# gyroflow/gyroflow

Hardware: NVIDIA H100
Metric: 4K frames/sec (fisheye+RS warp) (higher is better)
Workload: dtype f32

## Files before the change

gyroflow_b200/abi.py:

```python
import ctypes as C
import os

_HERE = os.path.dirname(os.path.abspath(__file__))
LIB_PATH = os.environ.get("GF_CUDA_LIB") or os.path.join(_HERE, "libgyroflow_cuda.so")

MATRIX_STRIDE = 14
MESH_MAX_LEN = 839
KERNEL_PARAMS_SIZE = 368


class KernelParams(C.Structure):
    _pack_ = 4
    _fields_ = [
        ("width", C.c_int32), ("height", C.c_int32), ("stride", C.c_int32),
        ("output_width", C.c_int32), ("output_height", C.c_int32), ("output_stride", C.c_int32),
        ("matrix_count", C.c_int32), ("interpolation", C.c_int32), ("background_mode", C.c_int32),
        ("flags", C.c_int32), ("bytes_per_pixel", C.c_int32), ("pix_element_count", C.c_int32),
        ("background", C.c_float * 4), ("f", C.c_float * 2), ("c", C.c_float * 2), ("k", C.c_float * 12),
        ("fov", C.c_float), ("r_limit", C.c_float), ("lens_correction_amount", C.c_float),
        ("input_vertical_stretch", C.c_float), ("input_horizontal_stretch", C.c_float),
        ("background_margin", C.c_float), ("background_margin_feather", C.c_float), ("canvas_scale", C.c_float),
        ("input_rotation", C.c_float), ("output_rotation", C.c_float),
        ("translation2d", C.c_float * 2), ("translation3d", C.c_float * 4),
        ("source_rect", C.c_int32 * 4), ("output_rect", C.c_int32 * 4),
# ... 136 lines not shown
    ("gf_lens_from_name", C.c_int, [C.c_char_p]),
    ("gf_lens_name", C.c_char_p, [C.c_int]),
    ("gf_pixel_bytes", C.c_int, [C.c_int]),
    ("gf_combo_supported", C.c_int, [C.c_int, C.c_int, C.c_int, C.c_int]),
    ("gf_cuda_create", C.c_int, [_P(C.c_void_p), C.c_int, _P(KernelParams), C.c_int, C.c_int, C.c_int,
                                 _P(BufferDesc), _P(BufferDesc), C.c_size_t]),
    ("gf_cuda_destroy", None, [C.c_void_p]),
    ("gf_cuda_undistort_image", C.c_int, [C.c_void_p, _P(BufferDesc), _P(BufferDesc), _P(KernelParams),
                                          C.c_void_p, C.c_size_t, C.c_void_p, C.c_size_t,
                                          C.c_void_p, C.c_size_t, C.c_void_p]),
    ("gf_cuda_undistort_image_dev", C.c_int, [C.c_void_p, _P(BufferDesc), _P(BufferDesc), _P(KernelParams),
                                              C.c_void_p, C.c_size_t, C.c_void_p, C.c_size_t, C.c_void_p]),
    ("gf_cuda_undistort_image_async", C.c_int, [C.c_void_p, _P(BufferDesc), _P(BufferDesc), _P(KernelParams),
                                                C.c_void_p, C.c_size_t, C.c_void_p, C.c_size_t, C.c_void_p]),
    ("gf_cuda_validate_tables_dev", C.c_int, [C.c_void_p, C.c_void_p, C.c_size_t]),
    ("gf_cuda_undistort_points", C.c_int, [C.c_void_p, C.c_void_p, C.c_int, C.c_int, C.c_double, C.c_size_t, C.c_int, C.c_double, C.c_void_p, C.c_size_t, C.c_void_p, C.c_void_p]),
    ("gf_cuda_stmap_distort_dev", C.c_int, [C.c_void_p, C.c_void_p, C.c_int, C.c_int, C.c_double, C.c_size_t, C.c_void_p, C.c_void_p]),
    ("gf_cuda_generate_stmap", C.c_int, [C.c_void_p, C.c_void_p, C.c_int, C.c_int, C.c_int, C.c_size_t, C.c_double, C.POINTER(C.c_int32), C.POINTER(C.c_int32),
                                          C.c_void_p, C.c_size_t, C.c_void_p, C.c_size_t, C.c_void_p]),
    ("gf_cuda_undistort_planes_dev", C.c_int, [C.c_void_p, C.c_size_t, C.c_void_p, C.c_void_p, C.c_void_p, C.c_void_p, C.c_size_t, C.c_void_p, C.c_size_t, C.c_void_p]),
    ("gf_cuda_undistort_planes", C.c_int, [C.c_void_p, C.c_size_t, C.c_void_p, C.c_void_p, C.c_void_p, C.c_void_p, C.c_size_t, C.c_void_p, C.c_size_t, C.c_void_p]),
    ("gf_cuda_selftest_exhaustive", C.c_int, [C.c_int, C.POINTER(C.c_ulonglong)]),
    ("gf_cuda_selftest_filter", C.c_int, [C.c_int, C.c_ulonglong, C.c_int, C.c_int, C.POINTER(C.c_ulonglong)]),
    ("gf_cuda_plan", C.c_int, [C.c_void_p, C.c_int, C.c_int, C.c_int, C.c_void_p, C.c_void_p, C.c_size_t, C.c_uint32, C.c_size_t]),
    ("gf_cuda_synchronize", C.c_int, [C.c_void_p]),
    ("gf_cuda_set_overlays", C.c_int, [C.c_void_p, C.c_int]),
    ("gf_cuda_last_error", C.c_char_p, [C.c_void_p]),
    ("gf_cuda_backend_name", C.c_char_p, []),
    ("gf_cuda_launch_count", C.c_uint64, [C.c_void_p]),
    ("gf_cuda_selftest", C.c_int, [C.c_int, C.c_ulonglong, C.c_ulonglong, _P(C.c_ulonglong)]),
    ("gf_frame_transform_at_timestamp", C.c_int, [_P(ComputeParams), C.c_double, C.c_size_t, _P(KernelParams), C.c_void_p, C.c_size_t,
                                                  _P(C.c_size_t), _P(C.c_double), _P(C.c_double)]),
    ("gf_cuda_gyro_upload", C.c_int, [_P(C.c_void_p), C.c_int, _P(ComputeParams)]),
    ("gf_cuda_gyro_free", None, [C.c_void_p]),
    ("gf_cuda_frame_transform_dev", C.c_int, [C.c_void_p, _P(ComputeParams), C.c_double, C.c_size_t, _P(KernelParams), C.c_void_p, C.c_size_t,
                                              _P(C.c_size_t), _P(C.c_double), _P(C.c_double), C.c_void_p]),
    ("gf_cuda_find_fovs", C.c_int, [C.c_void_p, _P(ComputeParams), C.c_int, C.c_int, C.c_void_p, C.c_size_t, C.c_float, C.c_void_p, C.c_void_p]),
    ("gf_zoom_dynamic_compute", C.c_int, [C.c_void_p, C.c_size_t, C.c_double, C.c_double, C.c_int, C.c_void_p]),
    ("gf_zoom_fovs", C.c_int, [_P(ZoomParams), C.c_void_p, C.c_void_p, C.c_size_t, C.c_void_p, C.c_void_p]),
    ("gf_cuda_calculate_fovs", C.c_int, [C.c_void_p, _P(ComputeParams), _P(ZoomParams), C.c_int, C.c_int, C.c_void_p, C.c_size_t,
                                         C.c_void_p, C.c_void_p, C.c_void_p]),
    ("gf_cuda_scan_tables_dev", C.c_int, [C.c_void_p, C.c_size_t, C.c_void_p, C.c_void_p]),
    ("gf_cuda_undistort_image_dev_flagged", C.c_int, [C.c_void_p, _P(BufferDesc), _P(BufferDesc), _P(KernelParams),
                                                      C.c_void_p, C.c_size_t, C.c_void_p, C.c_size_t, C.c_void_p, C.c_void_p]),
    ("gf_cuda_undistort_planes_dev_flagged", C.c_int, [C.c_void_p, C.c_size_t, C.c_void_p, C.c_void_p, C.c_void_p, C.c_void_p, C.c_size_t,
                                                       C.c_void_p, C.c_size_t, C.c_void_p, C.c_void_p]),
# ... 45 lines not shown
```

gyroflow_b200/csrc/c_abi.cu:

```cuda
#include <cuda_runtime.h>
#include <cstdio>
#include <cstring>
#include <cstdlib>
#include <mutex>
#include <cmath>
#include <algorithm>
#include <string>
#include <vector>

#include "kernel_registry.h"
#include "c_abi_internal.h"
#include <nvtx3/nvToolsExt.h>

using namespace gf;

namespace {

struct Slot {
    GrowBuf<float, true> h_mat, h_mesh;
    GrowBuf<float> d_mat, d_mesh;
    GrowBuf<double> d_mesh64;
    Event done;
};
constexpr int kSlots = 4;
// ... 165 lines not shown
    }
    A.feat = f;

    for (int i = 0; i < 4; ++i) A.bg[i] = p->background[i] * p->max_pixel_value;
    const float factor = fmaxf(1.0f - p->lens_correction_amount, 0.001f);
    A.out_c[0] = (float)p->output_width / 2.0f; A.out_c[1] = (float)p->output_height / 2.0f;
    A.out_f[0] = p->f[0] / p->fov / factor;      A.out_f[1] = p->f[1] / p->fov / factor;

    A.width_f = (float)p->width; A.height_f = (float)p->height;
    A.frame_w = A.width_f; A.frame_h = A.height_f;
    A.rot_cos = 1.0f; A.rot_sin = 0.0f;
    if (p->input_rotation != 0.0f) {
        const float rotation = p->input_rotation * (3.14159274101257324f / 180.0f);
        A.rot_cos = gf_cosf(rotation); A.rot_sin = gf_sinf(rotation);
        const float fx = A.rot_cos * (A.width_f - 0.0f) - A.rot_sin * (A.height_f - 0.0f) + 0.0f;
        const float fy = A.rot_sin * (A.width_f - 0.0f) + A.rot_cos * (A.height_f - 0.0f) + 0.0f;
        A.frame_w = rs_round(fabsf(fx)); A.frame_h = rs_round(fabsf(fy));
    }
    A.omap_x = make_map((float)p->output_rect[0], (float)(p->output_rect[0] + p->output_rect[2]), 0.0f, (float)p->output_width,  (float)A.out_cols);
    A.omap_y = make_map((float)p->output_rect[1], (float)(p->output_rect[1] + p->output_rect[3]), 0.0f, (float)p->output_height, (float)A.out_rows);
    A.smap_x = make_map(0.0f, A.frame_w, (float)p->source_rect[0], (float)(p->source_rect[0] + p->source_rect[2]), -1.0f);
    A.smap_y = make_map(0.0f, A.frame_h, (float)p->source_rect[1], (float)(p->source_rect[1] + p->source_rect[3]), -1.0f);
    A.rs_lim = (p->flags & 16) == 16 ? p->width : p->height;
    const float lim = p->pixel_value_limit;
    A.u8_limit = (lim != lim) ? 255 : (lim < 0.0f ? 0 : (lim >= 255.0f ? 255 : (int)lim));
    A.src_rect[0] = p->source_rect[0]; A.src_rect[1] = p->source_rect[1];
    A.src_rect[2] = p->source_rect[0] + p->source_rect[2]; A.src_rect[3] = p->source_rect[1] + p->source_rect[3];
    A.interior_span[0] = A.src_rect[2] - 2 - A.src_rect[0]; A.interior_span[1] = A.src_rect[3] - 2 - A.src_rect[1];
    if (A.interior_span[0] < 0 || A.interior_span[1] < 0 || A.interior_span[0] >= (1 << 17) || A.interior_span[1] >= (1 << 17) || A.rs_lim >= (1 << 22)) { A.interior_span[0] = 0; A.interior_span[1] = 0; A.feat |= F_WILD; }
    auto smap_ok = [](const MapC& m) { return m.fast_div && m.in_min == 0.0f && m.mul != 0.0f && tame(m.mul) && m.div > 0.0f && m.div <= 0x1p20f && std::isfinite(m.add) && fabsf(m.add) <= 0x1p16f; };
    if (!(smap_ok(A.smap_x) && smap_ok(A.smap_y) && fabsf(p->c[0]) >= 0x1p-10f && fabsf(p->c[1]) >= 0x1p-10f &&
          A.src_rect[0] >= 0 && A.src_rect[1] >= 0 && A.src_rect[2] <= (1 << 16) && A.src_rect[3] <= (1 << 16))) A.feat |= F_WILD;
    auto int_map_ok = [](const MapC& m) {
        return m.identity || (m.fast_div && m.mul > 0.0f && m.div > 0.0f && tame(m.mul) && std::isfinite(m.add) && fabsf(m.in_min) <= 0x1p20f);
    };
    if (!(int_map_ok(A.omap_x) && int_map_ok(A.omap_y))) A.feat |= F_WILD;
    A.hot.rect[0] = A.src_rect[0]; A.hot.rect[1] = A.src_rect[1]; A.hot.rect[2] = A.interior_span[0]; A.hot.rect[3] = A.interior_span[1];
    if (A.omap_x.identity && A.omap_y.identity && A.omap_x.add == truncf(A.omap_x.add) && A.omap_y.add == truncf(A.omap_y.add) &&
        fabsf(A.omap_x.add) < 0x1p20f && fabsf(A.omap_y.add) < 0x1p20f && fabsf(A.omap_x.in_min) < 0x1p20f && fabsf(A.omap_y.in_min) < 0x1p20f) {
        A.hot.x_off = (int)A.omap_x.add - (int)A.omap_x.in_min; A.hot.y_off = (int)A.omap_y.add - (int)A.omap_y.in_min;
        A.hot.x0 = std::max(0, -A.hot.x_off); A.hot.x1 = std::min(A.out_cols, p->output_width - A.hot.x_off);
        A.hot.y0 = std::max(0, -A.hot.y_off); A.hot.y1 = std::min(A.out_rows, p->output_height - A.hot.y_off);
        A.hot.full_rows = (int)std::min<size_t>(A.dst_len / (size_t)p->output_stride, (size_t)A.out_rows);
        const size_t tail = A.dst_len - (size_t)A.hot.full_rows * (size_t)p->output_stride;
        A.hot.last_cols = (A.hot.full_rows < A.out_rows) ? (int)std::min<size_t>(tail / (size_t)bpp, (size_t)A.out_cols) : 0;
        A.feat |= F_INTPRO;
    }
}

float filter_a_cap(const float* k) {
    auto B = [&](double t) { const double t2 = t * t; return t2 * (fabs((double)k[0]) + t2 * (fabs((double)k[1]) + t2 * (fabs((double)k[2]) + t2 * fabs((double)k[3])))); };
    for (int i = 0; i < 4; ++i) if (!std::isfinite(k[i])) return 0.0f;
    double lo = 0.0, hi = 1.55;
    if (B(hi) > 0.25) { for (int it = 0; it < 60; ++it) { const double mid = 0.5 * (lo + hi); if (B(mid) <= 0.25) lo = mid; else hi = mid; } }
    else lo = hi;
    if (lo < 0.5) return 0.0f;
    const double a = tan(lo) * tan(lo);
    return (float)std::min(a * 0.999, 16000.0);
}

struct FrameJob {
    const gf_buffer_desc* in; const gf_buffer_desc* out; const gf_kernel_params* p;
    const float* matrices; size_t matrix_rows;
    const float* mesh; size_t mesh_len;
    void* stream;
    bool tables_on_device = false;
    bool sync_host = true;
    size_t more_planes = 0;
// ... 604 lines not shown
```

gyroflow_b200/csrc/selftest.cu:

```cuda
#include <cuda_runtime.h>
#include <cstdio>
#include <cstdlib>
#include <cstring>
#include <cmath>
#include <vector>
#include "../../include/gyroflow_cuda.h"
#include "warp_kernel_x2.cuh"
#include "c_abi_internal.h"

using namespace gf;

namespace {
inline uint32_t __float_as_uint_host(float f) { uint32_t u; memcpy(&u, &f, 4); return u; }
__device__ __forceinline__ uint32_t mix(uint64_t v) {
    v ^= v >> 33; v *= 0xff51afd7ed558ccdULL; v ^= v >> 33; v *= 0xc4ceb9fe1a85ec53ULL; v ^= v >> 33;
    return (uint32_t)v;
}
__device__ __forceinline__ float gen(uint64_t i, uint32_t salt) {
    const uint32_t h = mix(i * 0x9E3779B97F4A7C15ULL + salt);
    const uint32_t sel = mix(i + 77u * salt) & 7u;
    if (sel < 3) return __uint_as_float(h);
    if (sel < 6) return __uint_as_float((h & 0x807fffffu) | ((100u + (mix(i ^ salt) % 56u)) << 23));
    return __uint_as_float((h & 0x007fffffu) | 0x3f800000u) - ((h >> 31) ? 0.0f : 1.0f);
}
// ... 92 lines not shown
    unsigned long long in_regime = 0, violations = 0, uncertain = 0; unsigned worst = 0;
    for (int ci = blockIdx.y; ci < n_cfg; ci += gridDim.y) {
        const FilterCfg C = cfgs[ci];
        gf_kernel_params P; memset(&P, 0, sizeof(P));
        for (int i = 0; i < 4; ++i) P.k[i] = C.k[i];
        P.f[0] = C.f1; P.f[1] = C.f1; P.c[0] = 0.5f * (float)C.w; P.c[1] = C.c1;
        const int nx = (C.w + step - 1) / step, ny = (C.h + step - 1) / step;
        for (int i = blockIdx.x * blockDim.x + threadIdx.x; i < nx * ny; i += gridDim.x * blockDim.x) {
            const float px = (float)((i % nx) * step + (ci % step)), py = (float)((i / nx) * step + ((ci / 3) % step));
            const float _x = (px * C.m[0] + py * C.m[1]) + C.m[2];
            const float _y = (px * C.m[3] + py * C.m[4]) + C.m[5];
            const float _w = (px * C.m[6] + py * C.m[7]) + C.m[8];
            float tvc;
            if (!Lens2<GF_LENS_OPENCV_FISHEYE>::approx_v(_x, _y, _w, P, C.a_cap, tvc)) continue;
            const float tv = tvc + P.c[1];
            if (!(fabsf(tv) < 0x1p20f)) continue;
            float ex, ey;
            Lens<GF_LENS_OPENCV_FISHEYE>::distort(_x, _y, _w, P, false, ex, ey);
            const float tv_exact = ey * P.f[1] + P.c[1];
            const float bound = __fmaf_rn(fabsf(tvc), rho, fabsf(tv) * 0x1p-22f);
            const float diff = fabsf(tv - tv_exact);
            ++in_regime;
            if (!(diff <= bound)) ++violations;
            const float z = tv - 0.5f;
            if (!(fabsf(z - ((z + 12582912.0f) - 12582912.0f)) > bound)) ++uncertain;
            const float ratio = bound > 0.0f ? diff / bound : (diff > 0.0f ? 1e9f : 0.0f);
            worst = max(worst, (unsigned)fminf(ratio * 1e6f, 4.0e9f));
        }
    }
    if (in_regime) atomicAdd(&out[0], in_regime);
    if (violations) atomicAdd(&out[1], violations);
    if (uncertain) atomicAdd(&out[2], uncertain);
    atomicMax(&out[3], (unsigned long long)worst);
}
}

extern "C" GF_API int gf_cuda_selftest_filter(int device, unsigned long long seed, int n_cfg, int step, unsigned long long* out4) {
    if (!out4 || n_cfg < 1 || step < 1) return GF_ERR_BAD_PARAMS;
    CK(nullptr, cudaSetDevice(device));
    std::vector<FilterCfg> cfgs((size_t)n_cfg);
    uint64_t st = seed * 0x9E3779B97F4A7C15ULL + 12345u;
    auto rnd = [&]() { st ^= st << 13; st ^= st >> 7; st ^= st << 17; return (double)(st >> 11) * (1.0 / 9007199254740992.0); };
    for (int i = 0; i < n_cfg; ++i) {
        FilterCfg& C = cfgs[(size_t)i];
        const int sizes[5][2] = { {3840, 2160}, {1920, 1080}, {7680, 4320}, {1280, 720}, {8192, 4320} };
        C.w = sizes[i % 5][0]; C.h = sizes[i % 5][1];
        double k[4]; for (int j = 0; j < 4; ++j) k[j] = (rnd() * 2.0 - 1.0) * pow(0.35, j);
        const double t_hit = 0.6 + 0.95 * rnd(), t2 = t_hit * t_hit;
// ... 6 lines not shown
        const double f = (0.3 + 0.9 * rnd()) * C.w, cx = 0.5 * C.w, cy = 0.5 * C.h;
        double ax[3] = { rnd() - 0.5, rnd() - 0.5, rnd() - 0.5 }; const double an = sqrt(ax[0]*ax[0] + ax[1]*ax[1] + ax[2]*ax[2]) + 1e-12;
        for (double& v : ax) v /= an;
        const double ang = 0.45 * rnd(), c = cos(ang), s = sin(ang), t = 1.0 - c;
        const double R[9] = { t*ax[0]*ax[0] + c, t*ax[0]*ax[1] - s*ax[2], t*ax[0]*ax[2] + s*ax[1],
                              t*ax[0]*ax[1] + s*ax[2], t*ax[1]*ax[1] + c, t*ax[1]*ax[2] - s*ax[0],
                              t*ax[0]*ax[2] - s*ax[1], t*ax[1]*ax[2] + s*ax[0], t*ax[2]*ax[2] + c };
        const double Ki[9] = { 1.0 / f, 0.0, -cx / f, 0.0, 1.0 / f, -cy / f, 0.0, 0.0, 1.0 };
        for (int r = 0; r < 3; ++r) for (int q = 0; q < 3; ++q) C.m[r * 3 + q] = (float)(R[0 * 3 + r] * Ki[0 * 3 + q] + R[1 * 3 + r] * Ki[1 * 3 + q] + R[2 * 3 + r] * Ki[2 * 3 + q]);
        C.f1 = (float)((0.3 + 0.9 * rnd()) * C.w); C.c1 = (float)(cy + (rnd() - 0.5) * 40.0);
    }
    GrowBuf<FilterCfg> d_cfg; GrowBuf<unsigned long long> d_out;
    CK(nullptr, d_cfg.reserve(cfgs.size(), nullptr));
    CK(nullptr, d_out.reserve(4, nullptr));
    CK(nullptr, cudaMemcpy(d_cfg.ptr, cfgs.data(), cfgs.size() * sizeof(FilterCfg), cudaMemcpyHostToDevice));
    CK(nullptr, cudaMemset(d_out.ptr, 0, 4 * sizeof(unsigned long long)));
    filter_check_kernel<<<dim3(132, (unsigned)(n_cfg < 64 ? n_cfg : 64)), 256>>>(d_cfg.ptr, n_cfg, step, 0x1p-17f, d_out.ptr);
    CK(nullptr, cudaGetLastError());
    CK(nullptr, cudaDeviceSynchronize());
    CK(nullptr, cudaMemcpy(out4, d_out.ptr, 4 * sizeof(unsigned long long), cudaMemcpyDeviceToHost));
    return GF_OK;
}

extern "C" GF_API int gf_cuda_selftest_exhaustive(int device, unsigned long long* out2) {
    if (!out2) return GF_ERR_BAD_PARAMS;
    CK(nullptr, cudaSetDevice(device));
    GrowBuf<unsigned long long> d;
    CK(nullptr, d.reserve(2, nullptr));
    CK(nullptr, cudaMemset(d.ptr, 0, 2 * sizeof(unsigned long long)));
    sweep_kernel<<<132 * 16, 256>>>(__float_as_uint_host(0x1p-28f), __float_as_uint_host(0x1p24f), 0, d.ptr);
    CK(nullptr, cudaGetLastError());
    sweep_kernel<<<132 * 16, 256>>>(__float_as_uint_host(0x1p-56f), __float_as_uint_host(0x1p48f), 1, d.ptr + 1);
    CK(nullptr, cudaGetLastError());
    CK(nullptr, cudaDeviceSynchronize());
    CK(nullptr, cudaMemcpy(out2, d.ptr, 2 * sizeof(unsigned long long), cudaMemcpyDeviceToHost));
    return GF_OK;
}

extern "C" GF_API int gf_cuda_selftest(int device, unsigned long long n, unsigned long long seed, unsigned long long* out4) {
    if (!out4) return GF_ERR_BAD_PARAMS;
    CK(nullptr, cudaSetDevice(device));
    GrowBuf<unsigned long long> d;
    CK(nullptr, d.reserve(4, nullptr));
    CK(nullptr, cudaMemset(d.ptr, 0, 4 * sizeof(unsigned long long)));
    GrowBuf<uint32_t> dbg;
    if (getenv("GF_SELFTEST_DEBUG")) { dbg.reserve(65, nullptr); cudaMemset(dbg.ptr, 0, 65 * 4); }
// ... 14 lines not shown
```

gyroflow_b200/csrc/warp_kernel.cuh:

```cuda
#pragma once
#include "lens_models.cuh"
#include "gf_coeffs_tables.h"
#include "f32x2.cuh"
#include <cuda_fp16.h>

namespace gf {

struct MapC {
    float in_min, mul, div, rcp, add;
    int   fast_div;
    int   identity;
};

__host__ __device__ inline MapC make_map(float in_min, float in_max, float out_min, float out_max, float max_abs_int_coord) {
    MapC m;
    m.in_min = in_min;
    m.mul = out_max - out_min;
    m.div = in_max - in_min;
    m.rcp = 1.0f / m.div;
    m.add = out_min;
    const float ad = fabsf(m.div);
    m.fast_div = (isfinite(m.div) && ad >= 0x1p-40f && ad <= 0x1p40f) ? 1 : 0;
    m.identity = (max_abs_int_coord >= 0.0f && m.mul == m.div && m.mul > 0.0f && in_min == truncf(in_min) &&
                  (max_abs_int_coord + fabsf(in_min)) * m.mul < 16777216.0f) ? 1 : 0;
// ... 7 lines not shown
    F_REFRACT    = 1u << 3,
    F_MESH       = 1u << 4,
    F_DIGITAL    = 1u << 5,
    F_HSTRETCH   = 1u << 6,
    F_VSTRETCH   = 1u << 7,
    F_LCA        = 1u << 8,
    F_INROT      = 1u << 9,
    F_BG1        = 1u << 10,
    F_BG2        = 1u << 11,
    F_BG3        = 1u << 12,
    F_FIXRANGE   = 1u << 13,
    F_FILLBG     = 1u << 14,
    F_LENS_NOOP  = 1u << 15,
    F_SRC_VEC    = 1u << 16,
    F_DST_VEC    = 1u << 17,
    F_FB_INV     = 1u << 18,
    F_IS_Y       = 1u << 19,
    F_T3D        = 1u << 20,
    F_PIXLIMIT   = 1u << 21,
    F_WILD       = 1u << 22,
    F_INTPRO     = 1u << 23,
    F_FILTER     = 1u << 24,
    F_SRC_VEC8   = 1u << 25,
};

constexpr uint32_t F_GENERAL_ONLY = F_HRS | F_RLIMIT | F_REFRACT | F_MESH | F_HSTRETCH | F_VSTRETCH | F_LCA | F_INROT |
                                    F_BG1 | F_BG2 | F_BG3 | F_FIXRANGE | F_FILLBG | F_LENS_NOOP | F_FB_INV | F_T3D | F_PIXLIMIT;
constexpr uint32_t F_LEAN_REQUIRED = F_SRC_VEC | F_DST_VEC;

template <bool GEN> __device__ __forceinline__ bool has(uint32_t feat, uint32_t bit) {
    if (GEN) return (feat & bit) != 0;
    if (bit & F_GENERAL_ONLY) return false;
    if (bit & (F_LEAN_REQUIRED | F_DIGITAL)) return true;
    return (feat & bit) != 0;
}

struct WarpArgs {
    gf_kernel_params p;
    const uint8_t* src;
    uint8_t*       dst;
    const float*   matrices;
    const float*   mesh;
    const double*  mesh64;
    const struct MeshAux* mesh_aux;
    uint2*         coord_out;
    const uint2*   coord_in;
// ... 3 lines not shown
        unsigned* count;
        unsigned* count_next;
        uint32_t  cap;
        int       tail;
        float     rho;
        float     a_cap;
    } flt;
    int            coord_shift;
    int            coord_maps;
    unsigned long long src_len, dst_len;
    int   mesh_len;
    int   out_rows;
    int   out_cols;
    uint32_t feat;
    float r_limit_sq;
    float out_c[2], out_f[2];
    float bg[4];
    MapC  omap_x, omap_y;
    MapC  smap_x, smap_y;
    float width_f, height_f;
    float frame_w, frame_h;
    float rot_cos, rot_sin;
    int   rs_lim;
    int   u8_limit;
    int   src_rect[4];
    int   interior_span[2];
    struct X2Hot {
        int x_off, y_off;
        int x0, x1, y0, y1;
        int full_rows, last_cols;
        int rect[4];
    } hot;
};

enum { SC_U8 = 0, SC_U16 = 1, SC_F32 = 2, SC_F16 = 3 };

template <int COUNT_, int SCALAR_> struct Pix {
    static constexpr int COUNT = COUNT_;
    static constexpr int SCALAR = SCALAR_;
    static constexpr int SBYTES = SCALAR_ == SC_U8 ? 1 : (SCALAR_ == SC_F32 ? 4 : 2);
    static constexpr int BYTES = COUNT_ * SBYTES;
    static constexpr bool POW2 = (BYTES == 1 || BYTES == 2 || BYTES == 4 || BYTES == 8 || BYTES == 16);
    static constexpr int ALIGN = POW2 ? BYTES : SBYTES;

    static GF_DEV float scalar_to_float(uint32_t raw) {
        if (SCALAR == SC_F32) return __uint_as_float(raw);
// ... 953 lines not shown
```

gyroflow_b200/csrc/warp_kernel_x2.cuh:

```cuda
#pragma once
#include "warp_kernel.cuh"
#include "approx_atan_table.inc"

namespace gf {

using p2::f2;

GF_DEV bool in_window_r2(float a) {
    const uint32_t t = (__float_as_uint(a) << 1) - (71u << 24);
    return t < (104u << 24);
}
GF_DEV bool zero_or_in_window(float v) {
    const uint32_t u = __float_as_uint(v) << 1;
    return u == 0u || (u - (67u << 24)) < (121u << 24);
}

template <int M> struct Lens2 { static constexpr bool kHas = false; };
template <int M> struct LensApprox { static constexpr bool value = false; };
template <> struct LensApprox<GF_LENS_OPENCV_FISHEYE> { static constexpr bool value = true; };

template <> struct Lens2<GF_LENS_OPENCV_FISHEYE> {
    static constexpr bool kHas = true;
    static GF_DEV bool approx_v(float _x, float _y, float _w, const gf_kernel_params& P, float a_cap, float& tvc) {
        const bool ok_w = (_w >= 0x1p-56f) & (_w < 0x1p48f);
        const float iw = p2::rcp_approx(_w);
        const float x = _x * iw, y = _y * iw;
        const float a = __fmaf_rn(x, x, y * y);
        const uint32_t ab = __float_as_uint(a);
        const int idx = min(max((int)(ab >> 19) - (int)GF_APX_BASE, 0), GF_APX_ROWS - 1);
        const float a0 = __uint_as_float((ab & 0xfff80000u) | 0x00040000u);
        const float4 c = __ldg(&GF_APX_TAB[idx]);
        const float d = a - a0;
        const float T = __fmaf_rn(d, __fmaf_rn(d, __fmaf_rn(d, c.w, c.z), c.y), c.x);
        const float t2 = (a * T) * T;
        const float s = __fmaf_rn(t2, __fmaf_rn(t2, __fmaf_rn(t2, __fmaf_rn(t2, P.k[3], P.k[2]), P.k[1]), P.k[0]), 1.0f);
        tvc = ((y * T) * s) * P.f[1];
        return ok_w & (a < a_cap);
    }
    template <bool TRUSTED>
    static GF_DEV void distort(f2 x, f2 y, f2 z, const gf_kernel_params& P, f2& ox, f2& oy, bool& bad) {
        using namespace p2;
        x = div_seq(x, z); y = div_seq(y, z);
        const f2 a = add(mul(x, x), mul(y, y));
        if (TRUSTED) {
            const float lo = fminf(fminf(z.x, z.y), fminf(a.x, a.y)), hi = fmaxf(fmaxf(z.x, z.y), fmaxf(a.x, a.y));
            bad |= !(lo >= 0x1p-56f) | !(hi < 0x1p48f);
        } else {
            bad |= !(z.x >= 0x1p-56f) | !(z.x < 0x1p48f) | !(z.y >= 0x1p-56f) | !(z.y < 0x1p48f) |
                   !in_window_r2(a.x) | !in_window_r2(a.y);
        }
        const f2 r = sqrt_seq(a);
        const f2 theta = atanf2_core(r, GF_ATAN_TAB);
// ... 368 lines not shown
GF_DEV float map_apply_int_lean(float x, const MapC& m) {
    if (m.identity) return (x - m.in_min) + m.add;
    const float a = (x - m.in_min) * m.mul;
    const float q0 = a * m.rcp;
    const float r0 = __fmaf_rn(-m.div, q0, a);
    return __fmaf_rn(r0, m.rcp, q0) + m.add;
}

GF_DEV int round_away_i32(float t) {
    const double h = __hiloint2double((int)((__float_as_uint(t) & 0x80000000u) | 0x3fe00000u), 0);
    const int r = __double2int_rz((double)t + h);
    return t == t ? r : 0;
}

template <bool BOUNDED = false>
GF_DEV void round_half_away_w(f2 a2, int& wa, int& wb) {
    const float sa = __fadd_rz(BOUNDED ? a2.x : fmaxf(a2.x, -4.0f), 8388608.0f);
    const float sb = __fadd_rz(BOUNDED ? a2.y : fmaxf(a2.y, -4.0f), 8388608.0f);
    wa = __float_as_int(sa) - 0x4affffff; wb = __float_as_int(sb) - 0x4affffff;
}
GF_DEV void round_away_clamped_x2(f2 t, int lim, int& ra, int& rb) {
    int wa, wb;
    round_half_away_w(p2::mul(t, p2::bc(2.0f)), wa, wb);
    ra = max(min(wa >> 1, lim), 0); rb = max(min(wb >> 1, lim), 0);
}

template <class PIX>
static __device__ __noinline__ void shade_cold(bool ok, float u, float v, const WarpArgs& A, uint8_t* __restrict__ out) {
    constexpr int C = PIX::COUNT;
    float pixel[C];
    if (ok) {
        sample_generic<2, PIX>(round_away_i32(u * 32.0f), round_away_i32(v * 32.0f), A, pixel);
    } else {
        #pragma unroll
        for (int ch = 0; ch < C; ++ch) pixel[ch] = A.bg[ch];
    }
    PIX::store(out, true, pixel);
}

template <class PIX>
GF_DEV void shade_lean(bool ok, bool far, float u, float v, int wu, int wv, const WarpArgs& A, uint8_t* __restrict__ out) {
    constexpr int C = PIX::COUNT;
    if (PIX::SCALAR == SC_U8) {
        const int sx0 = wu >> 1, sy0 = wv >> 1;
        const int sx = sx0 >> 5, sy = sy0 >> 5;
        const bool interior = ok & !far & ((unsigned)(sx - A.hot.rect[0]) <= (unsigned)A.hot.rect[2]) & ((unsigned)(sy - A.hot.rect[1]) <= (unsigned)A.hot.rect[3]);
        if (interior) {
            uint32_t N[C], s[C];
            sample_u8_bilinear<PIX>(sx0, sy0, A, N);
            #pragma unroll
            for (int ch = 0; ch < C; ++ch) s[ch] = N[ch] >> 10;
            PIX::store_scalars(out, true, s);
        } else {
            shade_cold<PIX>(ok, u, v, A, out);
        }
    } else {
        float pixel[C];
        if (ok) {
            sample_input_at<2, PIX, false>(u, v, A, pixel);
        } else {
            #pragma unroll
            for (int ch = 0; ch < C; ++ch) pixel[ch] = A.bg[ch];
        }
        PIX::store(out, true, pixel);
    }
}

#define GF_X2_ROWS_PER_BLOCK (2 * GF_BLOCK_Y)

template <int LENS, int DIGITAL, class PIX, bool TRUSTED, bool COORD>
GF_DEV void warp_x2_body(const WarpArgs& A, const int x, const int y0, const bool exact_prepass) {
    using namespace p2;
    const gf_kernel_params& P = A.p;
    if (x >= A.out_cols || y0 >= A.out_rows) return;
    const unsigned long long BYTES = COORD ? (unsigned long long)P.bytes_per_pixel : (unsigned long long)PIX::BYTES;
    const unsigned long long ostride = (unsigned long long)P.output_stride;
    const unsigned long long off_a = (unsigned long long)y0 * ostride + (unsigned long long)x * BYTES;
    const unsigned long long off_b = off_a + ostride;
    float opx, opy_a, opy_b;
    bool wr_a, wr_b;
    if (A.feat & F_INTPRO) {
        const bool in_x = (x >= A.hot.x0) & (x < A.hot.x1);
        const int y1 = y0 + 1;
        wr_a = in_x & (y0 >= A.hot.y0) & (y0 < A.hot.y1) & ((y0 < A.hot.full_rows) | ((y0 == A.hot.full_rows) & (x < A.hot.last_cols)));
        wr_b = in_x & (y1 >= A.hot.y0) & (y1 < A.hot.y1) & ((y1 < A.hot.full_rows) | ((y1 == A.hot.full_rows) & (x < A.hot.last_cols)));
        opx = (float)(x + A.hot.x_off); opy_a = (float)(y0 + A.hot.y_off); opy_b = (float)(y1 + A.hot.y_off);
    } else {
        opx = map_apply_int_lean((float)x, A.omap_x);
        opy_a = map_apply_int_lean((float)y0, A.omap_y);
        opy_b = map_apply_int_lean((float)(y0 + 1), A.omap_y);
        const bool in_x = (opx >= 0.0f) & (as_i32(opx) < P.output_width);
        wr_a = in_x & (off_a + BYTES <= A.dst_len) & (opy_a >= 0.0f) & (as_i32(opy_a) < P.output_height);
        wr_b = in_x & ((y0 + 1) < A.out_rows) & (off_b + BYTES <= A.dst_len) & (opy_b >= 0.0f) & (as_i32(opy_b) < P.output_height);
    }
    uint2* const cm_a = COORD ? A.coord_out + ((size_t)y0 * (size_t)A.out_cols + (size_t)x) : nullptr;
    const bool row_b = (y0 + 1) < A.out_rows;
    if (!(wr_a | wr_b)) {
        if (COORD) { *cm_a = make_uint2(GF_COORD_MARK, GF_COORD_SKIP); if (row_b) cm_a[A.out_cols] = make_uint2(GF_COORD_MARK, GF_COORD_SKIP); }
        return;
    }

    const float pxs = opx + P.translation2d[0];
    const f2 px = bc(pxs);
    const f2 py = mk(opy_a + P.translation2d[1], opy_b + P.translation2d[1]);
    const int lim = A.rs_lim;
    int sy_a, sy_b;
    round_away_clamped_x2(py, lim, sy_a, sy_b);
    bool have_row = false;
    if constexpr (TRUSTED && LensApprox<LENS>::value && DIGITAL == GF_LENS_NONE) if (!exact_prepass) {
        const MatRow9 rm = load_row9(A.matrices, (uint32_t)P.matrix_count / 2u);
        const float bx = pxs * rm.m01.x, by = pxs * rm.m23.y, bw = pxs * rm.m67.x;
        const float xa = (bx + py.x * rm.m01.y) + rm.m23.x, xb = (bx + py.y * rm.m01.y) + rm.m23.x;
        const float ya = (by + py.x * rm.m45.x) + rm.m45.y, yb = (by + py.y * rm.m45.x) + rm.m45.y;
        const float wa = (bw + py.x * rm.m67.y) + rm.m8,    wb = (bw + py.y * rm.m67.y) + rm.m8;
        float ca, cb;
        const bool ra = Lens2<LENS>::approx_v(xa, ya, wa, P, A.flt.a_cap, ca);
        const bool rb = Lens2<LENS>::approx_v(xb, yb, wb, P, A.flt.a_cap, cb);
        const float ta = ca + P.c[1], tb = cb + P.c[1];
        const float za = ta - 0.5f, zb = tb - 0.5f;
        const float da = fabsf(za - ((za + 12582912.0f) - 12582912.0f)), db = fabsf(zb - ((zb + 12582912.0f) - 12582912.0f));
        const float ea = __fmaf_rn(fabsf(ca), A.flt.rho, fabsf(ta) * 0x1p-22f), eb = __fmaf_rn(fabsf(cb), A.flt.rho, fabsf(tb) * 0x1p-22f);
        const bool sure = ra & rb & (da > ea) & (db > eb) & (fabsf(ta) < 0x1p20f) & (fabsf(tb) < 0x1p20f);
        if (sure) {
            round_away_clamped_x2(mk(ta, tb), lim, sy_a, sy_b);
            have_row = true;
        } else {
            const unsigned m = __activemask();
            const unsigned lane = threadIdx.x & 31u;
            const int leader = __ffs((int)m) - 1;
            unsigned base = 0;
            if ((int)lane == leader) base = atomicAdd(A.flt.count, (unsigned)__popc(m));
            base = __shfl_sync(m, base, leader);
            const unsigned slot = base + (unsigned)__popc(m & ((1u << lane) - 1u));
            if (slot < A.flt.cap) { A.flt.q[slot] = (uint32_t)x | ((uint32_t)(y0 >> 1) << 16); return; }
        }
    }
    if ((A.feat & F_RS) && !have_row) {
        const uint32_t mid = (uint32_t)P.matrix_count / 2u;
        f2 tu, tv; bool oa = true, ob = true, bad = false;
        rotate_and_distort_x2<LENS, DIGITAL, TRUSTED>(px, py, mid, mid, A, tu, tv, bad);
        if (bad) {
            const PairUV c = rotate_and_distort_cold<LENS, DIGITAL>(pxs, py.x, py.y, mid, mid, A, 0);
            oa = (c.ok & 1) != 0; ob = (c.ok & 2) != 0; tv = mk(c.va, c.vb);
        }
        int ra, rb;
        round_away_clamped_x2(tv, lim, ra, rb);
        sy_a = oa ? ra : sy_a; sy_b = ob ? rb : sy_b;
    }
    const uint32_t last = (uint32_t)(P.matrix_count - 1);
    const uint32_t idx_a = min((uint32_t)sy_a, last), idx_b = min((uint32_t)sy_b, last);
    f2 u, v; bool ok_a = true, ok_b = true, far_a = false, far_b = false, bad = false;
    rotate_and_distort_x2<LENS, DIGITAL, TRUSTED>(px, py, idx_a, idx_b, A, u, v, bad);
    u = map_apply_x2(u, A.smap_x, bad);
    v = map_apply_x2(v, A.smap_y, bad);
    if (bad) {
        const PairUV c = rotate_and_distort_cold<LENS, DIGITAL>(pxs, py.x, py.y, idx_a, idx_b, A, 1);
        ok_a = (c.ok & 1) != 0; ok_b = (c.ok & 2) != 0; far_a = (c.ok & 4) != 0; far_b = (c.ok & 8) != 0;
        u = mk(c.ua, c.ub); v = mk(c.va, c.vb);
    }

    if (COORD) {
        *cm_a = !wr_a ? make_uint2(GF_COORD_MARK, GF_COORD_SKIP) : (ok_a ? make_uint2(__float_as_uint(u.x), __float_as_uint(v.x)) : make_uint2(GF_COORD_MARK, GF_COORD_NONE));
        if (row_b) cm_a[A.out_cols] = !wr_b ? make_uint2(GF_COORD_MARK, GF_COORD_SKIP) : (ok_b ? make_uint2(__float_as_uint(u.y), __float_as_uint(v.y)) : make_uint2(GF_COORD_MARK, GF_COORD_NONE));
        return;
    }
    int wu_a = 0, wu_b = 0, wv_a = 0, wv_b = 0;
    if (PIX::SCALAR == SC_U8) {
        round_half_away_w<true>(mul(u, bc(64.0f)), wu_a, wu_b);
        round_half_away_w<true>(mul(v, bc(64.0f)), wv_a, wv_b);
    }
    if (wr_a) shade_lean<PIX>(ok_a, far_a, u.x, v.x, wu_a, wv_a, A, A.dst + off_a);
    if (wr_b) shade_lean<PIX>(ok_b, far_b, u.y, v.y, wu_b, wv_b, A, A.dst + off_b);
}

template <int LENS, int DIGITAL, class PIX, int MINB, bool COORD = false>
__global__ void __launch_bounds__(GF_BLOCK_X * GF_BLOCK_Y, MINB)
warp_kernel_x2(const __grid_constant__ WarpArgs A) {
    constexpr bool kFilter = LensApprox<LENS>::value && DIGITAL == GF_LENS_NONE;
    asm volatile("griddepcontrol.wait;" ::: "memory");
    const bool trusted = __ldg(A.table_flags) == 0u;
    if constexpr (kFilter) if (A.flt.tail) {
        const unsigned tid = (blockIdx.y * gridDim.x + blockIdx.x) * (blockDim.x * blockDim.y) + threadIdx.y * blockDim.x + threadIdx.x;
        if (tid == 0u) *A.flt.count_next = 0u;
        if (!trusted) return;
        const unsigned n = min(*A.flt.count, A.flt.cap);
        const unsigned stride = gridDim.x * gridDim.y * blockDim.x * blockDim.y;
        for (unsigned i = tid; i < n; i += stride) {
            const uint32_t e = A.flt.q[i];
            warp_x2_body<LENS, DIGITAL, PIX, true, COORD>(A, (int)(e & 0xffffu), (int)(e >> 16) * 2, true);
        }
        return;
    }
    const int x = blockIdx.x * GF_BLOCK_X + threadIdx.x;
    const int y0 = (blockIdx.y * blockDim.y + threadIdx.y) * 2;
    if (trusted) warp_x2_body<LENS, DIGITAL, PIX, true, COORD>(A, x, y0, !(kFilter && (A.feat & F_FILTER)));
// ... 5 lines not shown
```

include/gyroflow_cuda.h:

```cpp
#ifndef GYROFLOW_CUDA_H
#define GYROFLOW_CUDA_H

#include <stddef.h>
#include <stdint.h>

#ifdef __cplusplus
extern "C" {
#endif

#if defined(_WIN32)
#  define GF_API __declspec(dllexport)
#else
#  define GF_API __attribute__((visibility("default")))
#endif

#pragma pack(push, 4)
typedef struct gf_kernel_params {
    int32_t width;
    int32_t height;
    int32_t stride;
    int32_t output_width;
    int32_t output_height;
    int32_t output_stride;
    int32_t matrix_count;
// ... 183 lines not shown

GF_API int         gf_cuda_scan_tables_dev(const float* matrices_dev, size_t matrix_rows, uint32_t* table_flags_dev, void* cu_stream);
GF_API int         gf_cuda_undistort_image_dev_flagged(gf_cuda_ctx* ctx, const gf_buffer_desc* in, const gf_buffer_desc* out,
                                                       const gf_kernel_params* params, const float* matrices_dev, size_t matrix_rows,
                                                       const float* mesh_dev, size_t mesh_len, const uint32_t* table_flags_dev, void* cu_stream);
GF_API int         gf_cuda_undistort_planes_dev_flagged(gf_cuda_ctx* ctx, size_t n_planes, const gf_buffer_desc* in, const gf_buffer_desc* out,
                                                        const gf_kernel_params* params, const float* matrices_dev, size_t matrix_rows,
                                                        const float* mesh_dev, size_t mesh_len, const uint32_t* table_flags_dev, void* cu_stream);
GF_API int         gf_cuda_validate_tables_dev(gf_cuda_ctx* ctx, const float* matrices_dev, size_t matrix_rows);

GF_API int         gf_cuda_plan(const gf_kernel_params* params, int pixel_type, int distortion_model, int digital_lens,
                                const gf_buffer_desc* in, const gf_buffer_desc* out, size_t mesh_len, uint32_t table_flags, size_t n_planes);

GF_API int         gf_cuda_set_overlays(gf_cuda_ctx* ctx, int enabled);

GF_API int         gf_cuda_synchronize(gf_cuda_ctx* ctx);
GF_API const char* gf_cuda_last_error(gf_cuda_ctx* ctx);
GF_API const char* gf_cuda_backend_name(void);
GF_API uint64_t    gf_cuda_launch_count(gf_cuda_ctx* ctx);

GF_API int         gf_cuda_selftest(int device, unsigned long long n, unsigned long long seed, unsigned long long* out4);
GF_API int         gf_cuda_selftest_exhaustive(int device, unsigned long long* out2);
GF_API int         gf_cuda_selftest_filter(int device, unsigned long long seed, int n_cfg, int step, unsigned long long* out4);


typedef struct gf_quat_track {
    const int64_t* ts_us;
    const double*  quats;
    size_t         n;
} gf_quat_track;

typedef struct gf_keyframe_track { const int64_t* ts_us; const double* value; const uint8_t* easing; size_t n; } gf_keyframe_track;
enum { GF_KF_FOV = 0, GF_KF_VIDEO_ROTATION, GF_KF_ZOOMING_CENTER_X, GF_KF_ZOOMING_CENTER_Y, GF_KF_BACKGROUND_MARGIN, GF_KF_BACKGROUND_FEATHER,
       GF_KF_LENS_CORRECTION_STRENGTH, GF_KF_LIGHT_REFRACTION_COEFF, GF_KF_COUNT };
GF_API int gf_keyframe_value_at(const gf_keyframe_track* track, double timestamp_ms, double timestamp_scale, double* out);

typedef struct gf_compute_params {
    int32_t width, height, output_width, output_height;
    double  camera_matrix[9];
    double  distortion_coeffs[12];
    double  radial_distortion_limit;
    double  input_horizontal_stretch, input_vertical_stretch;
    double  fov_scale;
    const double* fovs;          size_t n_fovs;
    const double* minimal_fovs;  size_t n_minimal_fovs;
    double  lens_optimal_fov;    int32_t has_optimal_fov;
// ... 132 lines not shown
```

Baseline: 8054.

## Streamline warp_x2 hot path: certify_row helper, cold finish path, short-row flag

Restructures the per-pixel warp body by folding row rounding and clamping into a certify_row helper using __vimin_s32_relu, precomputing row_lim on the host, and moving the rare invalid-coordinate handling into a noinline cold function so the hot path always shades with ok=true. The partial-last-row write checks now run only when a new F_SHORTROW flag is set, with hot.y1 tightened on the host otherwise. The aim is fewer instructions and registers in the common path. It also adds a certify selftest entry point, and the changed rounding and fallback logic carries some correctness risk.

```diff
diff --git a/gyroflow_b200/abi.py b/gyroflow_b200/abi.py
--- a/gyroflow_b200/abi.py
+++ b/gyroflow_b200/abi.py
@@ -182,6 +182,7 @@
     ("gf_cuda_undistort_planes", C.c_int, [C.c_void_p, C.c_size_t, C.c_void_p, C.c_void_p, C.c_void_p, C.c_void_p, C.c_size_t, C.c_void_p, C.c_size_t, C.c_void_p]),
     ("gf_cuda_selftest_exhaustive", C.c_int, [C.c_int, C.POINTER(C.c_ulonglong)]),
     ("gf_cuda_selftest_filter", C.c_int, [C.c_int, C.c_ulonglong, C.c_int, C.c_int, C.POINTER(C.c_ulonglong)]),
+    ("gf_cuda_selftest_certify", C.c_int, [C.c_int, C.c_void_p, C.c_size_t, C.c_float, C.c_int, C.c_void_p, C.c_void_p]),
     ("gf_cuda_plan", C.c_int, [C.c_void_p, C.c_int, C.c_int, C.c_int, C.c_void_p, C.c_void_p, C.c_size_t, C.c_uint32, C.c_size_t]),
     ("gf_cuda_synchronize", C.c_int, [C.c_void_p]),
     ("gf_cuda_set_overlays", C.c_int, [C.c_void_p, C.c_int]),
diff --git a/gyroflow_b200/csrc/c_abi.cu b/gyroflow_b200/csrc/c_abi.cu
--- a/gyroflow_b200/csrc/c_abi.cu
+++ b/gyroflow_b200/csrc/c_abi.cu
@@ -211,6 +211,7 @@
     A.smap_x = make_map(0.0f, A.frame_w, (float)p->source_rect[0], (float)(p->source_rect[0] + p->source_rect[2]), -1.0f);
     A.smap_y = make_map(0.0f, A.frame_h, (float)p->source_rect[1], (float)(p->source_rect[1] + p->source_rect[3]), -1.0f);
     A.rs_lim = (p->flags & 16) == 16 ? p->width : p->height;
+    A.row_lim = std::min(A.rs_lim, p->matrix_count - 1);
     const float lim = p->pixel_value_limit;
     A.u8_limit = (lim != lim) ? 255 : (lim < 0.0f ? 0 : (lim >= 255.0f ? 255 : (int)lim));
     A.src_rect[0] = p->source_rect[0]; A.src_rect[1] = p->source_rect[1];
@@ -233,6 +234,11 @@
         A.hot.full_rows = (int)std::min<size_t>(A.dst_len / (size_t)p->output_stride, (size_t)A.out_rows);
         const size_t tail = A.dst_len - (size_t)A.hot.full_rows * (size_t)p->output_stride;
         A.hot.last_cols = (A.hot.full_rows < A.out_rows) ? (int)std::min<size_t>(tail / (size_t)bpp, (size_t)A.out_cols) : 0;
+        if (A.hot.full_rows < A.out_rows) {
+            if (A.hot.last_cols >= A.hot.x1) A.hot.y1 = std::min(A.hot.y1, A.hot.full_rows + 1);
+            else if (A.hot.last_cols <= A.hot.x0) A.hot.y1 = std::min(A.hot.y1, A.hot.full_rows);
+            else A.feat |= F_SHORTROW;
+        }
         A.feat |= F_INTPRO;
     }
 }
diff --git a/gyroflow_b200/csrc/selftest.cu b/gyroflow_b200/csrc/selftest.cu
--- a/gyroflow_b200/csrc/selftest.cu
+++ b/gyroflow_b200/csrc/selftest.cu
@@ -138,8 +138,8 @@
             const float diff = fabsf(tv - tv_exact);
             ++in_regime;
             if (!(diff <= bound)) ++violations;
-            const float z = tv - 0.5f;
-            if (!(fabsf(z - ((z + 12582912.0f) - 12582912.0f)) > bound)) ++uncertain;
+            int row;
+            if (!certify_row(tv, bound, C.h, row)) ++uncertain;
             const float ratio = bound > 0.0f ? diff / bound : (diff > 0.0f ? 1e9f : 0.0f);
             worst = max(worst, (unsigned)fminf(ratio * 1e6f, 4.0e9f));
         }
@@ -192,6 +192,31 @@
     return GF_OK;
 }
 
+namespace {
+__global__ void certify_kernel(const float* __restrict__ t, size_t n, float eps, int lim, uint8_t* __restrict__ cert, int32_t* __restrict__ row) {
+    for (size_t i = blockIdx.x * (size_t)blockDim.x + threadIdx.x; i < n; i += (size_t)gridDim.x * blockDim.x) {
+        int r;
+        cert[i] = certify_row(t[i], eps, lim, r) ? 1 : 0;
+        row[i] = r;
+    }
+}
+}
+
+extern "C" GF_API int gf_cuda_selftest_certify(int device, const float* t, size_t n, float eps, int lim, uint8_t* cert_out, int32_t* row_out) {
+    if (!t || !cert_out || !row_out) return GF_ERR_BAD_PARAMS;
+    if (n == 0) return GF_OK;
+    CK(nullptr, cudaSetDevice(device));
+    GrowBuf<float> d_t; GrowBuf<uint8_t> d_c; GrowBuf<int32_t> d_r;
+    CK(nullptr, d_t.reserve(n, nullptr)); CK(nullptr, d_c.reserve(n, nullptr)); CK(nullptr, d_r.reserve(n, nullptr));
+    CK(nullptr, cudaMemcpy(d_t.ptr, t, n * sizeof(float), cudaMemcpyHostToDevice));
+    certify_kernel<<<132 * 8, 256>>>(d_t.ptr, n, eps, lim, d_c.ptr, d_r.ptr);
+    CK(nullptr, cudaGetLastError());
+    CK(nullptr, cudaDeviceSynchronize());
+    CK(nullptr, cudaMemcpy(cert_out, d_c.ptr, n, cudaMemcpyDeviceToHost));
+    CK(nullptr, cudaMemcpy(row_out, d_r.ptr, n * sizeof(int32_t), cudaMemcpyDeviceToHost));
+    return GF_OK;
+}
+
 extern "C" GF_API int gf_cuda_selftest_exhaustive(int device, unsigned long long* out2) {
     if (!out2) return GF_ERR_BAD_PARAMS;
     CK(nullptr, cudaSetDevice(device));
diff --git a/gyroflow_b200/csrc/warp_kernel.cuh b/gyroflow_b200/csrc/warp_kernel.cuh
--- a/gyroflow_b200/csrc/warp_kernel.cuh
+++ b/gyroflow_b200/csrc/warp_kernel.cuh
@@ -53,6 +53,7 @@
     F_INTPRO     = 1u << 23,
     F_FILTER     = 1u << 24,
     F_SRC_VEC8   = 1u << 25,
+    F_SHORTROW   = 1u << 26,
 };
 
 constexpr uint32_t F_GENERAL_ONLY = F_HRS | F_RLIMIT | F_REFRACT | F_MESH | F_HSTRETCH | F_VSTRETCH | F_LCA | F_INROT |
@@ -102,6 +103,7 @@
     float frame_w, frame_h;
     float rot_cos, rot_sin;
     int   rs_lim;
+    int   row_lim;
     int   u8_limit;
     int   src_rect[4];
     int   interior_span[2];
diff --git a/gyroflow_b200/csrc/warp_kernel_x2.cuh b/gyroflow_b200/csrc/warp_kernel_x2.cuh
--- a/gyroflow_b200/csrc/warp_kernel_x2.cuh
+++ b/gyroflow_b200/csrc/warp_kernel_x2.cuh
@@ -27,7 +27,7 @@
         const float x = _x * iw, y = _y * iw;
         const float a = __fmaf_rn(x, x, y * y);
         const uint32_t ab = __float_as_uint(a);
-        const int idx = min(max((int)(ab >> 19) - (int)GF_APX_BASE, 0), GF_APX_ROWS - 1);
+        const int idx = __vimin_s32_relu((int)(ab >> 19) - (int)GF_APX_BASE, GF_APX_ROWS - 1);
         const float a0 = __uint_as_float((ab & 0xfff80000u) | 0x00040000u);
         const float4 c = __ldg(&GF_APX_TAB[idx]);
         const float d = a - a0;
@@ -442,7 +442,15 @@
 GF_DEV void round_away_clamped_x2(f2 t, int lim, int& ra, int& rb) {
     int wa, wb;
     round_half_away_w(p2::mul(t, p2::bc(2.0f)), wa, wb);
-    ra = max(min(wa >> 1, lim), 0); rb = max(min(wb >> 1, lim), 0);
+    ra = __vimin_s32_relu(wa >> 1, lim); rb = __vimin_s32_relu(wb >> 1, lim);
+}
+
+GF_DEV bool certify_row(float t, float eps, int lim, int& row) {
+    const float s = __fadd_rn(t, 12582912.0f);
+    const float r = __fsub_rn(t, __fsub_rn(s, 12582912.0f));
+    const float d = __fsub_rd(0.5f, fabsf(r));
+    row = __vimin_s32_relu(__float_as_int(s) - 0x4b400000, lim);
+    return (d > eps) & (fabsf(t) < 0x1p20f);
 }
 
 template <class PIX>
@@ -488,6 +496,27 @@
 
 #define GF_X2_ROWS_PER_BLOCK (2 * GF_BLOCK_Y)
 
+template <int LENS, int DIGITAL, class PIX, bool COORD>
+static __device__ __noinline__ void finish_pair_cold(const WarpArgs& A, int x, int y0, float pxs, f2 py, uint32_t idx_a, uint32_t idx_b,
+                                                     bool wr_a, bool wr_b) {
+    const PairUV c = rotate_and_distort_cold<LENS, DIGITAL>(pxs, py.x, py.y, idx_a, idx_b, A, 1);
+    const bool ok_a = (c.ok & 1) != 0, ok_b = (c.ok & 2) != 0;
+    if (COORD) {
+        uint2* const cm_a = A.coord_out + ((size_t)y0 * (size_t)A.out_cols + (size_t)x);
+        *cm_a = !wr_a ? make_uint2(GF_COORD_MARK, GF_COORD_SKIP) : (ok_a ? make_uint2(__float_as_uint(c.ua), __float_as_uint(c.va)) : make_uint2(GF_COORD_MARK, GF_COORD_NONE));
+        if ((y0 + 1) < A.out_rows) cm_a[A.out_cols] = !wr_b ? make_uint2(GF_COORD_MARK, GF_COORD_SKIP) : (ok_b ? make_uint2(__float_as_uint(c.ub), __float_as_uint(c.vb)) : make_uint2(GF_COORD_MARK, GF_COORD_NONE));
+        return;
+    }
+    const unsigned long long off_a = (unsigned long long)y0 * (unsigned long long)A.p.output_stride + (unsigned long long)x * (unsigned long long)PIX::BYTES;
+    int wu_a = 0, wu_b = 0, wv_a = 0, wv_b = 0;
+    if (PIX::SCALAR == SC_U8) {
+        round_half_away_w<true>(p2::mul(p2::mk(c.ua, c.ub), p2::bc(64.0f)), wu_a, wu_b);
+        round_half_away_w<true>(p2::mul(p2::mk(c.va, c.vb), p2::bc(64.0f)), wv_a, wv_b);
+    }
+    if (wr_a) shade_lean<PIX>(ok_a, (c.ok & 4) != 0, c.ua, c.va, wu_a, wv_a, A, A.dst + off_a);
+    if (wr_b) shade_lean<PIX>(ok_b, (c.ok & 8) != 0, c.ub, c.vb, wu_b, wv_b, A, A.dst + off_a + (unsigned long long)A.p.output_stride);
+}
+
 template <int LENS, int DIGITAL, class PIX, bool TRUSTED, bool COORD>
 GF_DEV void warp_x2_body(const WarpArgs& A, const int x, const int y0, const bool exact_prepass) {
     using namespace p2;
@@ -500,10 +529,14 @@
     float opx, opy_a, opy_b;
     bool wr_a, wr_b;
     if (A.feat & F_INTPRO) {
+        const int y1 = y0 + 1;
         const bool in_x = (x >= A.hot.x0) & (x < A.hot.x1);
-        const int y1 = y0 + 1;
-        wr_a = in_x & (y0 >= A.hot.y0) & (y0 < A.hot.y1) & ((y0 < A.hot.full_rows) | ((y0 == A.hot.full_rows) & (x < A.hot.last_cols)));
-        wr_b = in_x & (y1 >= A.hot.y0) & (y1 < A.hot.y1) & ((y1 < A.hot.full_rows) | ((y1 == A.hot.full_rows) & (x < A.hot.last_cols)));
+        wr_a = in_x & (y0 >= A.hot.y0) & (y0 < A.hot.y1);
+        wr_b = in_x & (y1 >= A.hot.y0) & (y1 < A.hot.y1);
+        if (A.feat & F_SHORTROW) {
+            wr_a &= (y0 < A.hot.full_rows) | ((y0 == A.hot.full_rows) & (x < A.hot.last_cols));
+            wr_b &= (y1 < A.hot.full_rows) | ((y1 == A.hot.full_rows) & (x < A.hot.last_cols));
+        }
         opx = (float)(x + A.hot.x_off); opy_a = (float)(y0 + A.hot.y_off); opy_b = (float)(y1 + A.hot.y_off);
     } else {
         opx = map_apply_int_lean((float)x, A.omap_x);
@@ -523,65 +556,53 @@
     const float pxs = opx + P.translation2d[0];
     const f2 px = bc(pxs);
     const f2 py = mk(opy_a + P.translation2d[1], opy_b + P.translation2d[1]);
-    const int lim = A.rs_lim;
-    int sy_a, sy_b;
-    round_away_clamped_x2(py, lim, sy_a, sy_b);
-    bool have_row = false;
-    if constexpr (TRUSTED && LensApprox<LENS>::value && DIGITAL == GF_LENS_NONE) if (!exact_prepass) {
-        const MatRow9 rm = load_row9(A.matrices, (uint32_t)P.matrix_count / 2u);
-        const float bx = pxs * rm.m01.x, by = pxs * rm.m23.y, bw = pxs * rm.m67.x;
-        const float xa = (bx + py.x * rm.m01.y) + rm.m23.x, xb = (bx + py.y * rm.m01.y) + rm.m23.x;
-        const float ya = (by + py.x * rm.m45.x) + rm.m45.y, yb = (by + py.y * rm.m45.x) + rm.m45.y;
-        const float wa = (bw + py.x * rm.m67.y) + rm.m8,    wb = (bw + py.y * rm.m67.y) + rm.m8;
-        float ca, cb;
-        const bool ra = Lens2<LENS>::approx_v(xa, ya, wa, P, A.flt.a_cap, ca);
-        const bool rb = Lens2<LENS>::approx_v(xb, yb, wb, P, A.flt.a_cap, cb);
-        const float ta = ca + P.c[1], tb = cb + P.c[1];
-        const float za = ta - 0.5f, zb = tb - 0.5f;
-        const float da = fabsf(za - ((za + 12582912.0f) - 12582912.0f)), db = fabsf(zb - ((zb + 12582912.0f) - 12582912.0f));
-        const float ea = __fmaf_rn(fabsf(ca), A.flt.rho, fabsf(ta) * 0x1p-22f), eb = __fmaf_rn(fabsf(cb), A.flt.rho, fabsf(tb) * 0x1p-22f);
-        const bool sure = ra & rb & (da > ea) & (db > eb) & (fabsf(ta) < 0x1p20f) & (fabsf(tb) < 0x1p20f);
-        if (sure) {
-            round_away_clamped_x2(mk(ta, tb), lim, sy_a, sy_b);
-            have_row = true;
+    const int lim = A.row_lim;
+    int sy_a = 0, sy_b = 0;
+    do {
+        if constexpr (TRUSTED && LensApprox<LENS>::value && DIGITAL == GF_LENS_NONE) {
+            if (!exact_prepass) {
+                const MatRow9 rm = load_row9(A.matrices, (uint32_t)P.matrix_count / 2u);
+                const float bx = pxs * rm.m01.x, by = pxs * rm.m23.y, bw = pxs * rm.m67.x;
+                const float xa = (bx + py.x * rm.m01.y) + rm.m23.x, xb = (bx + py.y * rm.m01.y) + rm.m23.x;
+                const float ya = (by + py.x * rm.m45.x) + rm.m45.y, yb = (by + py.y * rm.m45.x) + rm.m45.y;
+                const float wa = (bw + py.x * rm.m67.y) + rm.m8,    wb = (bw + py.y * rm.m67.y) + rm.m8;
+                float ca, cb;
+                const bool ra = Lens2<LENS>::approx_v(xa, ya, wa, P, A.flt.a_cap, ca);
+                const bool rb = Lens2<LENS>::approx_v(xb, yb, wb, P, A.flt.a_cap, cb);
+                const float ta = ca + P.c[1], tb = cb + P.c[1];
+                const float ea = __fmaf_rn(fabsf(ca), A.flt.rho, fabsf(ta) * 0x1p-22f), eb = __fmaf_rn(fabsf(cb), A.flt.rho, fabsf(tb) * 0x1p-22f);
+                const bool ca_ok = certify_row(ta, ea, lim, sy_a), cb_ok = certify_row(tb, eb, lim, sy_b);
+                if (ra & rb & ca_ok & cb_ok) break;
+                const unsigned m = __activemask();
+                const unsigned lane = threadIdx.x & 31u;
+                const int leader = __ffs((int)m) - 1;
+                unsigned base = 0;
+                if ((int)lane == leader) base = atomicAdd(A.flt.count, (unsigned)__popc(m));
+                base = __shfl_sync(m, base, leader);
+                const unsigned slot = base + (unsigned)__popc(m & ((1u << lane) - 1u));
+                if (slot < A.flt.cap) { A.flt.q[slot] = (uint32_t)x | ((uint32_t)(y0 >> 1) << 16); return; }
+            } else if (!(A.feat & F_RS)) break;
         } else {
-            const unsigned m = __activemask();
-            const unsigned lane = threadIdx.x & 31u;
-            const int leader = __ffs((int)m) - 1;
-            unsigned base = 0;
-            if ((int)lane == leader) base = atomicAdd(A.flt.count, (unsigned)__popc(m));
-            base = __shfl_sync(m, base, leader);
-            const unsigned slot = base + (unsigned)__popc(m & ((1u << lane) - 1u));
-            if (slot < A.flt.cap) { A.flt.q[slot] = (uint32_t)x | ((uint32_t)(y0 >> 1) << 16); return; }
-        }
-    }
-    if ((A.feat & F_RS) && !have_row) {
+            if (!(A.feat & F_RS)) break;
+        }
         const uint32_t mid = (uint32_t)P.matrix_count / 2u;
-        f2 tu, tv; bool oa = true, ob = true, bad = false;
+        f2 tu, tv; bool bad = false;
         rotate_and_distort_x2<LENS, DIGITAL, TRUSTED>(px, py, mid, mid, A, tu, tv, bad);
         if (bad) {
             const PairUV c = rotate_and_distort_cold<LENS, DIGITAL>(pxs, py.x, py.y, mid, mid, A, 0);
-            oa = (c.ok & 1) != 0; ob = (c.ok & 2) != 0; tv = mk(c.va, c.vb);
-        }
-        int ra, rb;
-        round_away_clamped_x2(tv, lim, ra, rb);
-        sy_a = oa ? ra : sy_a; sy_b = ob ? rb : sy_b;
-    }
-    const uint32_t last = (uint32_t)(P.matrix_count - 1);
-    const uint32_t idx_a = min((uint32_t)sy_a, last), idx_b = min((uint32_t)sy_b, last);
-    f2 u, v; bool ok_a = true, ok_b = true, far_a = false, far_b = false, bad = false;
-    rotate_and_distort_x2<LENS, DIGITAL, TRUSTED>(px, py, idx_a, idx_b, A, u, v, bad);
+            tv = mk((c.ok & 1) ? c.va : py.x, (c.ok & 2) ? c.vb : py.y);
+        }
+        round_away_clamped_x2(tv, lim, sy_a, sy_b);
+    } while (false);
+    f2 u, v; bool bad = false;
+    rotate_and_distort_x2<LENS, DIGITAL, TRUSTED>(px, py, (uint32_t)sy_a, (uint32_t)sy_b, A, u, v, bad);
     u = map_apply_x2(u, A.smap_x, bad);
     v = map_apply_x2(v, A.smap_y, bad);
-    if (bad) {
-        const PairUV c = rotate_and_distort_cold<LENS, DIGITAL>(pxs, py.x, py.y, idx_a, idx_b, A, 1);
-        ok_a = (c.ok & 1) != 0; ok_b = (c.ok & 2) != 0; far_a = (c.ok & 4) != 0; far_b = (c.ok & 8) != 0;
-        u = mk(c.ua, c.ub); v = mk(c.va, c.vb);
-    }
+    if (bad) { finish_pair_cold<LENS, DIGITAL, PIX, COORD>(A, x, y0, pxs, py, (uint32_t)sy_a, (uint32_t)sy_b, wr_a, wr_b); return; }
 
     if (COORD) {
-        *cm_a = !wr_a ? make_uint2(GF_COORD_MARK, GF_COORD_SKIP) : (ok_a ? make_uint2(__float_as_uint(u.x), __float_as_uint(v.x)) : make_uint2(GF_COORD_MARK, GF_COORD_NONE));
-        if (row_b) cm_a[A.out_cols] = !wr_b ? make_uint2(GF_COORD_MARK, GF_COORD_SKIP) : (ok_b ? make_uint2(__float_as_uint(u.y), __float_as_uint(v.y)) : make_uint2(GF_COORD_MARK, GF_COORD_NONE));
+        *cm_a = !wr_a ? make_uint2(GF_COORD_MARK, GF_COORD_SKIP) : make_uint2(__float_as_uint(u.x), __float_as_uint(v.x));
+        if (row_b) cm_a[A.out_cols] = !wr_b ? make_uint2(GF_COORD_MARK, GF_COORD_SKIP) : make_uint2(__float_as_uint(u.y), __float_as_uint(v.y));
         return;
     }
     int wu_a = 0, wu_b = 0, wv_a = 0, wv_b = 0;
@@ -589,8 +610,8 @@
         round_half_away_w<true>(mul(u, bc(64.0f)), wu_a, wu_b);
         round_half_away_w<true>(mul(v, bc(64.0f)), wv_a, wv_b);
     }
-    if (wr_a) shade_lean<PIX>(ok_a, far_a, u.x, v.x, wu_a, wv_a, A, A.dst + off_a);
-    if (wr_b) shade_lean<PIX>(ok_b, far_b, u.y, v.y, wu_b, wv_b, A, A.dst + off_b);
+    if (wr_a) shade_lean<PIX>(true, false, u.x, v.x, wu_a, wv_a, A, A.dst + off_a);
+    if (wr_b) shade_lean<PIX>(true, false, u.y, v.y, wu_b, wv_b, A, A.dst + off_b);
 }
 
 template <int LENS, int DIGITAL, class PIX, int MINB, bool COORD = false>
diff --git a/include/gyroflow_cuda.h b/include/gyroflow_cuda.h
--- a/include/gyroflow_cuda.h
+++ b/include/gyroflow_cuda.h
@@ -229,6 +229,7 @@
 GF_API int         gf_cuda_selftest(int device, unsigned long long n, unsigned long long seed, unsigned long long* out4);
 GF_API int         gf_cuda_selftest_exhaustive(int device, unsigned long long* out2);
 GF_API int         gf_cuda_selftest_filter(int device, unsigned long long seed, int n_cfg, int step, unsigned long long* out4);
+GF_API int         gf_cuda_selftest_certify(int device, const float* t, size_t n, float eps, int lim, uint8_t* cert_out, int32_t* row_out);
 
 
 typedef struct gf_quat_track {
```

New measurement: 8719, median of 6. 8.3% higher.
